# wq2012/SpectralCluster

Measured on AMD Instinct MI355X. Metric: predict() calls/sec, n=8192 d=256 ICASSP2018 (GraphCut, eigengap k in [2,20], cosine k-means), higher is better.
Workload: dtype f64; 1 GPU; icassp2018_graphcut_n8192_d256_k8_max20; n_samples=8192, n_features=256, parallelism=replicas x1, collectives=none

## Files before the change

### include/spectralcluster_amd.h

```cpp
#ifndef SPECTRALCLUSTER_AMD_H_
#define SPECTRALCLUSTER_AMD_H_

#include <stddef.h>
#include <stdint.h>

#ifdef __cplusplus
extern "C" {
#endif

#define SC_ABI_VERSION 11
#define SC_MAX_OPS 16
#define SC_MAX_BLUR_RADIUS 32
#define SC_MAX_EIG 128
#define SC_MAX_STAGES 16

typedef struct sc_handle_s* sc_handle;

typedef enum sc_status {
  SC_OK = 0,
  SC_ERR_INVALID = -1,
  SC_ERR_OOM = -2,
  SC_ERR_HIP = -3,
  SC_ERR_NOT_CONVERGED = -4,
  SC_ERR_UNSUPPORTED = -5,
// ... 134 lines not shown
enum { SC_MEM_HOST = 0, SC_MEM_DEVICE = 1 };
typedef struct sc_array {
  const void* data;
  int32_t dtype;
  int32_t location;
  int64_t rows, cols;
  int64_t row_stride;
  int64_t col_stride;
} sc_array;
int sc_array_layout(int* array_bytes, int* field_offsets);
int sc_device_count(void);
int sc_device_info(int device, char* name, int name_len, char* arch, int arch_len,
                   int* compute_units, int64_t* total_mem_bytes);

int sc_create(int device, sc_handle* out);
int sc_destroy(sc_handle h);
int sc_reserve(sc_handle h, int n_max, int d_max);
const char* sc_last_error(sc_handle h);
int sc_synchronize(sc_handle h);
void* sc_stream(sc_handle h);
int sc_set_profiling(sc_handle h, int level);
int sc_set_diffuse_mode(sc_handle h, int mode);
int sc_set_free_prune(sc_handle h, int on);

int sc_config_default(sc_config* cfg);
int sc_gaussian_weights(double sigma, int32_t* radius, double* weights);
int sc_set_blur_weights(sc_handle h, int radius, const double* weights);

int sc_predict(sc_handle h, const double* x, int n, int d, const sc_config* cfg,
               int64_t* labels, sc_diag* diag);

int sc_predict_array(sc_handle h, const sc_array* x, const sc_config* cfg, int64_t* labels,
                     sc_diag* diag);

int sc_set_embeddings(sc_handle h, const double* x, int n, int d);
int sc_set_embeddings_array(sc_handle h, const sc_array* x);
int sc_compute_affinity(sc_handle h);
int sc_set_affinity(sc_handle h, const double* affinity, int n);
int sc_set_affinity_array(sc_handle h, const sc_array* affinity);
int sc_predict_affinity_array(sc_handle h, const sc_array* affinity, const sc_config* cfg,
                              int64_t* labels, sc_diag* diag);
int sc_eig_ncluster(sc_handle h, const sc_config* cfg, sc_diag* diag);
int sc_num_eigenvalues(sc_handle h);
int sc_get_eigenvalues(sc_handle h, double* out, int count);
int sc_num_eigenvectors(sc_handle h);
int sc_get_eigenvectors(sc_handle h, double* out, int n, int ncols);
// ... 360 lines not shown
```

### spectralcluster_amd/_lib.py

```python

from __future__ import annotations

import ctypes
import os
import threading
import typing

import numpy as np

SC_MAX_OPS = 16
SC_MAX_BLUR_RADIUS = 32
SC_MAX_EIG = 128
SC_MAX_STAGES = 16

SC_OK = 0
SC_ERR_INVALID = -1
SC_ERR_OOM = -2
SC_ERR_HIP = -3
SC_ERR_NOT_CONVERGED = -4
SC_ERR_UNSUPPORTED = -5
SC_ERR_NON_FINITE = -6

STAGE_NAMES = ("affinity", "refine", "diffuse", "scaling", "eig", "kmeans",
               "total", "blur", "threshold_sym", "matvec", "affinity_gemm",
# ... 183 lines not shown

_c_int64_p = ctypes.POINTER(ctypes.c_int64)
_c_int_p = ctypes.POINTER(ctypes.c_int)
_handle_t = ctypes.c_void_p

PROTOTYPES = {
    "sc_abi_version": (ctypes.c_int, []),
    "sc_struct_sizes": (ctypes.c_int, [ctypes.POINTER(ctypes.c_int),
                                       ctypes.POINTER(ctypes.c_int)]),
    "sc_array_layout": (ctypes.c_int, [ctypes.POINTER(ctypes.c_int),
                                       ctypes.POINTER(ctypes.c_int)]),
    "sc_device_count": (ctypes.c_int, []),
    "sc_device_info": (ctypes.c_int, [ctypes.c_int, ctypes.c_char_p, ctypes.c_int,
                                      ctypes.c_char_p, ctypes.c_int, _c_int_p,
                                      _c_int64_p]),
    "sc_create": (ctypes.c_int, [ctypes.c_int, ctypes.POINTER(_handle_t)]),
    "sc_destroy": (ctypes.c_int, [_handle_t]),
    "sc_reserve": (ctypes.c_int, [_handle_t, ctypes.c_int, ctypes.c_int]),
    "sc_last_error": (ctypes.c_char_p, [_handle_t]),
    "sc_synchronize": (ctypes.c_int, [_handle_t]),
    "sc_set_profiling": (ctypes.c_int, [_handle_t, ctypes.c_int]),
    "sc_set_diffuse_mode": (ctypes.c_int, [_handle_t, ctypes.c_int]),
    "sc_set_free_prune": (ctypes.c_int, [_handle_t, ctypes.c_int]),
    "sc_stage_diffuse_rowstats": (ctypes.c_int, [_handle_t, _c_double_p, ctypes.c_int,
                                                 ctypes.c_int, _c_double_p, _c_double_p,
                                                 ctypes.POINTER(ctypes.c_int32)]),
    "sc_stage_block_operator": (ctypes.c_int, [_handle_t, ctypes.c_int,
                                               ctypes.POINTER(ctypes.c_int32),
                                               ctypes.POINTER(_c_double_p),
                                               ctypes.POINTER(_c_double_p),
                                               ctypes.POINTER(_c_double_p),
                                               ctypes.POINTER(_c_double_p),
                                               ctypes.POINTER(_c_double_p),
                                               ctypes.POINTER(_c_double_p), ctypes.c_int]),
    "sc_stage_krylov_state": (ctypes.c_int, [_handle_t, ctypes.POINTER(ctypes.c_int32),
                                             _c_double_p, _c_double_p, _c_double_p, _c_double_p,
                                             _c_double_p]),
    "sc_stage_front": (ctypes.c_int, [_handle_t, ctypes.c_int, ctypes.POINTER(ScConfig),
                                      ctypes.c_int, ctypes.POINTER(ctypes.c_int32), ctypes.c_int,
                                      ctypes.POINTER(_c_double_p), _c_double_p, _c_double_p,
                                      ctypes.POINTER(ScFrontOut)]),
    "sc_stage_tridiag": (ctypes.c_int, [_handle_t, _c_double_p, ctypes.c_int, _c_double_p,
                                        _c_double_p, _c_double_p, _c_double_p, _c_double_p,
                                        _c_double_p]),
    "sc_stage_tridiag_values": (ctypes.c_int, [_handle_t, _c_double_p, _c_double_p, ctypes.c_int,
                                               _c_double_p]),
# ... 561 lines not shown
```

### spectralcluster_amd/csrc/api.hip

```cpp
#include <algorithm>
#include <array>
#include <cmath>
#include <cstdio>
#include <cstdlib>
#include <cstring>
#include <vector>

#include <condition_variable>
#include <mutex>
#include <string>
#include <thread>

#include "handle.h"
#include "host_pool.h"

int ensure_matrices(sc_handle h, int n, int d, bool affinity_copy) {
  h->krylov_m = 0;
  h->arnoldi_m = 0;
  const size_t ldn = matrix_ld(n);
  const size_t nn = (size_t)n * ldn * sizeof(double);
  if (affinity_copy) SC_TRY(grow(h, h->A0, nn));
  SC_TRY(grow(h, h->B1, nn));
  SC_TRY(grow(h, h->B2, nn));
  if (d > 0) {
// ... 116 lines not shown
  hipDeviceProp_t prop;
  if (hipGetDeviceProperties(&prop, device) != hipSuccess) return SC_ERR_HIP;
  if (name && name_len > 0) snprintf(name, name_len, "%s", prop.name);
  if (arch && arch_len > 0) snprintf(arch, arch_len, "%s", prop.gcnArchName);
  if (compute_units) *compute_units = prop.multiProcessorCount;
  if (total_mem_bytes) *total_mem_bytes = (int64_t)prop.totalGlobalMem;
  return SC_OK;
}


extern "C" int sc_create(int device, sc_handle* out) {
  if (!out) return SC_ERR_INVALID;
  *out = nullptr;
  int count = 0;
  if (hipGetDeviceCount(&count) != hipSuccess || count <= 0) return SC_ERR_HIP;
  if (device < 0 || device >= count) return SC_ERR_INVALID;
  sc_handle h = new sc_handle_s();
  h->device = device;
  if (hipSetDevice(device) != hipSuccess ||
      hipStreamCreateWithFlags(&h->stream, hipStreamNonBlocking) != hipSuccess) {
    delete h;
    return SC_ERR_HIP;
  }
  const unsigned ev_flags = hipEventDisableSystemFence;
  for (int i = 0; i < 48; ++i) {
    if (hipEventCreateWithFlags(&h->ev[i], ev_flags) != hipSuccess) {
      delete h;
      return SC_ERR_HIP;
    }
  }
  if (hipHostMalloc(reinterpret_cast<void**>(&h->h_theta), 3 * kLdq * sizeof(double)) !=
          hipSuccess ||
      hipHostMalloc(reinterpret_cast<void**>(&h->h_flags), 16 * sizeof(int)) !=
          hipSuccess ||
      hipHostMalloc(reinterpret_cast<void**>(&h->h_rr),
                    (2 * kHostRRSingle * kHostRRSingle + 64) * sizeof(double)) != hipSuccess) {
    delete h;
    return SC_ERR_HIP;
  }
  *out = h;
  return SC_OK;
}

extern "C" int sc_destroy(sc_handle h) {
  if (!h) return SC_OK;
  for (sc_handle sub : h->pool) sc_destroy(sub);
  h->pool.clear();
  for (sc_handle sub : h->gslots) sc_destroy(sub);
  h->gslots.clear();
  for (sc_handle sub : h->gshort) sc_destroy(sub);
  h->gshort.clear();
  hipSetDevice(h->device);
  hipStreamSynchronize(h->stream);
  DevBuf* bufs[] = {&h->X,     &h->Xn,    &h->A0,     &h->B1,      &h->B2,    &h->rowmax,
                    &h->rowsum, &h->cvec,  &h->pvec,   &h->tvec,    &h->deg,   &h->blurw, &h->blur_tmp, &h->dvec, &h->cut, &h->rmpart, &h->splitk, &h->tilemap, &h->tilemap_table, &h->cropval, &h->statp, &h->crvec, &h->thetai, &h->Vre, &h->Vim, &h->gpart, &h->gsrc, &h->genL, &h->ahc_size, &h->ahc_chain, &h->ahc_Z, &h->ahc_lab, &h->ahc_cent, &h->fb_part, &h->fb_small, &h->sck_slots, &h->sck_part, &h->sck_rec, &h->sck_mats, &h->fb_x, &h->fb_cent, &h->fb_int, &h->Cq, &h->Cband, &h->Cpairs, &h->Cporig, &h->cp[0], &h->cp[1], &h->cp[2], &h->cp[3], &h->cp[4], &h->symflag,
                    &h->Q,     &h->Q2,    &h->Vs,     &h->W,       &h->partial, &h->T,
                    &h->Y,     &h->Yt,    &h->theta,  &h->resid,   &h->G,     &h->Rinv,
                    &h->Hbuf,  &h->hsq,   &h->colnorm, &h->flags,  &h->E,     &h->Ek,   &h->Eio,
                    &h->td_d,  &h->td_e,  &h->td_theta, &h->td_work, &h->td_tau, &h->td_panel, &h->mvsym,
                    &h->kXc,   &h->kxsq,  &h->kclosest, &h->kcand, &h->kenorm, &h->krnd,
                    &h->kcent, &h->klab32, &h->klab64, &h->kinfo, &h->kchain, &h->gkrnd, &h->gpack, &h->gypack, &h->ginfo, &h->glabels, &h->gjtab, &h->gsftab, &h->gswtab,
                    &h->kbig, &h->kbigw, &h->fq, &h->ft32, &h->fy1, &h->fR, &h->fscal, &h->fwords, &h->fcand, &h->fY, &h->fsplit, &h->fypart, &h->frpart, &h->fq2part, &h->fmx64, &h->ftau64, &h->fplan, &h->Xalt, &h->Xstage, &h->gneg};
  for (DevBuf* b : bufs)
    if (b->p) hipFree(b->p);
  for (DevBuf& b : h->kgen)
    if (b.p) hipFree(b.p);
  for (int i = 0; i < 48; ++i) hipEventDestroy(h->ev[i]);
  if (h->h_theta) hipHostFree(h->h_theta);
  if (h->h_flags) hipHostFree(h->h_flags);
  if (h->h_rr) hipHostFree(h->h_rr);
  if (h->h_free) hipHostFree(h->h_free);
  if (h->h_reduce) hipHostFree(h->h_reduce);
  if (h->h_sck) hipHostFree(h->h_sck);
  if (h->sync_ev) hipEventDestroy(h->sync_ev);
  for (int b = 0; b < kGroupBanks; ++b) {
    if (h->gbank_ev[b]) hipEventDestroy(h->gbank_ev[b]);
    if (h->gbank_stream[b]) hipStreamDestroy(h->gbank_stream[b]);
  }
  if (h->gchain_stream) hipStreamDestroy(h->gchain_stream);
  if (h->copy_stream) hipStreamDestroy(h->copy_stream);
  if (h->gcheck_ev) hipEventDestroy(h->gcheck_ev);
  for (sc_handle lane : h->glanes) sc_destroy(lane);
  h->glanes.clear();
  delete h->gpool;
  if (h->h_gpack) hipHostFree(h->h_gpack);
  if (h->h_gypack) hipHostFree(h->h_gypack);
  if (h->h_gjtab) hipHostFree(h->h_gjtab);
  if (h->h_gsftab) hipHostFree(h->h_gsftab);
  if (h->h_gswtab) hipHostFree(h->h_gswtab);
  if (h->gsftab_ev) hipEventDestroy(h->gsftab_ev);
  if (h->h_ginfo) hipHostFree(h->h_ginfo);
  if (h->h_glabels) hipHostFree(h->h_glabels);
  hipStreamDestroy(h->stream);
  delete h;
  return SC_OK;
}

extern "C" const char* sc_last_error(sc_handle h) { return h ? h->err.c_str() : ""; }

extern "C" int sc_synchronize(sc_handle h) {
  if (!h) return SC_ERR_INVALID;
  SC_HIP(h, hipStreamSynchronize(h->stream));
  return SC_OK;
}

extern "C" int sc_reserve(sc_handle h, int n_max, int d_max) {
  if (!h || n_max <= 0 || d_max < 0) return SC_ERR_INVALID;
  SC_HIP(h, hipSetDevice(h->device));
  SC_TRY(ensure_matrices(h, n_max, d_max));
  SC_TRY(ensure_eig(h, n_max));
  SC_TRY(ensure_kmeans(h, n_max));
  return SC_OK;
}

static double numpy_sum_short(const double* a, int n) {
// ... 334 lines not shown
  t.pending = false;
  if (!diag) return;
  float dms = 0.f;
  for (int i = 0; i < t.n_diffuse; ++i) dms += ev_ms(h, t.diffuse[i][0], t.diffuse[i][1]);
  diag->stage_ms[SC_STAGE_DIFFUSE] = dms;
  diag->stage_ms[SC_STAGE_REFINE] = ev_ms(h, t.begin, t.after_refine) - dms;
  diag->stage_ms[SC_STAGE_SCALING] = ev_ms(h, t.after_refine, t.after_scaling);
  diag->stage_ms[SC_STAGE_EIG] = ev_ms(h, t.after_scaling, t.after_eig);
  if (t.free_path) {
    diag->stage_ms[SC_STAGE_FREE_QUANTIZE] = ev_ms(h, h->free_ev[0], h->free_ev[1]);
    diag->stage_ms[SC_STAGE_FREE_PRODUCT] = ev_ms(h, h->free_ev[1], h->free_ev[2]);
    diag->stage_ms[SC_STAGE_FREE_SCAN] = ev_ms(h, h->free_ev[2], h->free_ev[3]);
    diag->stage_ms[SC_STAGE_FREE_STATS] = ev_ms(h, h->free_ev[3], h->free_ev[4]);
  }
  if (t.fine) {
    diag->stage_ms[SC_STAGE_BLUR] = ev_ms(h, t.blur[0], t.blur[1]);
    diag->stage_ms[SC_STAGE_THRESHOLD_SYM] = ev_ms(h, t.thr[0], t.thr[1]);
    float mv = 0.f;
    for (int i = 0; i < h->n_mv_ev; ++i) mv += ev_ms(h, h->mv_ev[i][0], h->mv_ev[i][1]);
    diag->stage_ms[SC_STAGE_MATVEC] = mv;
  }
}

int eig_ncluster_impl(sc_handle h, const sc_config* cfg, sc_diag* diag, FrontResult* front_only,
                      const FrontResult* resume, bool defer_timing,
                      FrontResult* stop_before_solver) {
  const int n = h->n, ld = h->ldn;
  hipStream_t s = h->stream;
  const double* cur = ptr<double>(h->A0);
  double* bufs[2] = {ptr<double>(h->B1), ptr<double>(h->B2)};
  int which = 0;
  bool symmetric = h->affinity_symmetric;
  const bool constrain_after = constraint_active(h, cfg, false);
  bool folded_rownorm = false;
  int e_begin, e_after_refine;
  const bool fine = h->profile_level >= 2;
  int eb0 = -1, eb1 = -1, et0 = -1, et1 = -1;
  h->n_mv_ev = 0;
  bool free_path = false;
  const double* amax_of = nullptr;
  const double* digits_of = nullptr;
  float diffuse_ms_events[SC_MAX_OPS][2];
  int n_diffuse = 0;
  ev_rec(h, &e_begin);
  const bool blur_fast = (cfg->blur_radius == 4 || cfg->blur_radius == 8) && n >= 128;
  const double* pending_diag = nullptr;
  bool have_partials = false;
  bool have_row_stats = false;
  int crop_source = 0, cut_kernel = 0;
  h->last_blur = BlurLaunch();
  if (resume) {
    cur = resume->matrix;
    symmetric = resume->symmetric;
    folded_rownorm = resume->folded_rownorm;
    which = resume->scratch == bufs[0] ? 0 : 1;
    if (resume->free_op) h->free_checked = false;
  }
  for (int i = 0; i < (resume ? 0 : cfg->n_ops); ++i) {
    const int op = cfg->ops[i];
    const int next = i + 1 < cfg->n_ops ? cfg->ops[i + 1] : 0;
    const int next2 = i + 2 < cfg->n_ops ? cfg->ops[i + 2] : 0;
    const bool thr_sym_fusable = true;
    const bool partials_usable = cfg->threshold_type == SC_THRESHOLD_ROW_MAX &&
                                 !cfg->preserve_diagonal;
    if (op == SC_OP_ROW_WISE_NORMALIZE && symmetric && i == cfg->n_ops - 1 &&
        !constrain_after) {
      folded_rownorm = true;
// ... 135 lines not shown
    double* out = bufs[which];
    which ^= 1;
    SC_TRY(adjust_affinity(h, cfg, cur, symmetric, out, n, ld));
    cur = out;
    symmetric = symmetric && h->constraint_symmetric;
    have_row_stats = false;
  }
  ev_rec(h, &e_after_refine);
  bool flags_by_kernel = false;
  if (resume) {
    SC_TRY(ensure_eig(h, n));
  } else if (!symmetric) {
    SC_TRY(ensure_gen(h, n));
    launch_row_stats(s, cur, n, ld, ptr<double>(h->rowmax), ptr<double>(h->deg));
    launch_scaling_general(s, ptr<double>(h->deg), n, cfg->laplacian_type,
                           ptr<double>(h->cvec), ptr<double>(h->crvec), ptr<double>(h->pvec));
  } else {
    if (!have_row_stats)
      launch_row_stats(s, cur, n, ld, ptr<double>(h->rowmax), ptr<double>(h->rowsum));
    SC_TRY(ensure_eig(h, n));
    launch_scaling_vectors(s, ptr<double>(h->rowmax), ptr<double>(h->rowsum), n,
                           cfg->laplacian_type, folded_rownorm ? 1 : 0, ptr<double>(h->cvec),
                           ptr<double>(h->pvec), ptr<double>(h->tvec), ptr<int>(h->flags),
                           h->affinity_from_embeddings ? ptr<int>(h->symflag) : nullptr);
    flags_by_kernel = true;
  }
  SC_TRY(ensure_eig(h, n));
  if (flags_by_kernel) {
  } else if (h->affinity_from_embeddings)
    SC_HIP(h, hipMemcpyAsync(ptr<int>(h->flags) + 12, ptr<int>(h->symflag) + 1, sizeof(int),
                             hipMemcpyDeviceToDevice, s));
  else
    SC_HIP(h, hipMemsetAsync(ptr<int>(h->flags) + 12, 0, sizeof(int), s));
  launch_check_finite(s, ptr<double>(h->cvec), ptr<double>(h->pvec), n, ptr<int>(h->flags) + 12);
  if (front_only && !flags_by_kernel)
    SC_HIP(h, hipMemsetAsync(ptr<int>(h->flags) + 13, 0, 3 * sizeof(int), s));
  SC_TRY(check_last(h, "scaling launch"));
  if (sw::eig_trace() > 2 && symmetric) {
    std::vector<double> rm(n), rs(n);
    hipMemcpyAsync(rm.data(), h->rowmax.p, n * sizeof(double), hipMemcpyDeviceToHost, s);
    hipMemcpyAsync(rs.data(), h->rowsum.p, n * sizeof(double), hipMemcpyDeviceToHost, s);
    hipStreamSynchronize(s);
    int imin = 0, imax = 0;
    for (int i = 0; i < n; ++i) {
      if (rm[i] < rm[imin]) imin = i;
      if (rm[i] > rm[imax]) imax = i;
    }
    fprintf(stderr, "[sc] scaling: fused stats %d; rowmax min %.6g at %d, max %.6g at %d; "
            "rowsum[%d] %.6g\n", (int)have_row_stats, rm[imin], imin, rm[imax], imax, imin,
            rs[imin]);
  }
  int e_after_scaling;
  ev_rec(h, &e_after_scaling);
  FrontResult op;
  op.matrix = cur;
  op.scratch = bufs[which];
  op.ld = ld;
  op.symmetric = symmetric;
  op.folded_rownorm = folded_rownorm;
  op.free_op = free_path || (resume && resume->free_op);
  op.laplacian_type = cfg->laplacian_type;
  op.chain_flags_cleared = flags_by_kernel;
  op.skip_fused = resume && resume->skip_fused;
  op.digits_fused = free_path && digits_of == cur;
  op.diffuse_explicit = !free_path && n_diffuse > 0;
  op.crop_source = crop_source;
  op.cut_kernel = cut_kernel;
  if (stop_before_solver) {
    *stop_before_solver = op;
    return SC_OK;
  }
  if (front_only) {
    *front_only = op;
    return SC_OK;
  }
  EigRequest rq = make_eig_request(cfg);
  EigDecision dc;
  std::vector<double> w;
  if (symmetric) {
    SC_TRY(sym_topk(h, op, n, rq, diag, &dc, &w));
  } else {
    rq.decision_aware = 1;
    SC_TRY(gen_topk(h, cur, ld, n, cfg->laplacian_type, rq, diag, &dc, &w, bufs[which]));
  }
  int e_after_eig;
  ev_rec(h, &e_after_eig);
  h->last_w = w;
  if (diag) {
    diag->n = n;
    diag->n_clusters_raw = dc.n_clusters_raw;
    diag->max_delta = dc.max_delta;
    diag->eig_descending = rq.descend;
    diag->n_eigenvalues = std::min((int)w.size(), SC_MAX_EIG);
    for (int i = 0; i < diag->n_eigenvalues; ++i) diag->eigenvalues[i] = w[i];
    diag->symmetry_state = !symmetric ? 3 : (folded_rownorm ? 2 : 1);
    if (!free_path && n_diffuse > 0) diag->diffuse_path = SC_DIFFUSE_PATH_EXPLICIT;
  }
  StageEvents& t = h->stage_events;
// ... 69 lines not shown
  sc_diag* dg = diag ? diag : &local;
  memset(dg, 0, sizeof(*dg));
  h->nev = 0;
  int e0, e1, e2;
  ev_rec(h, &e0);
  if (from_embeddings) SC_TRY(sc_compute_affinity(h));
  if (constraint_active(h, cfg, true)) SC_TRY(sc_apply_constraint(h, cfg));
  ev_rec(h, &e1);
  SC_TRY(eig_ncluster_impl(h, cfg, dg, nullptr, nullptr, true));
  int k = dg->n_clusters_raw;
  if (cfg->min_clusters > 0 && k < cfg->min_clusters) k = cfg->min_clusters;
  const int rc_cluster = sc_cluster(h, cfg, k, labels, dg);
  if (rc_cluster != SC_OK) {
    h->stage_events.pending = false;
    return rc_cluster;
  }
  ev_rec(h, &e2);
  SC_HIP(h, hipStreamSynchronize(h->stream));
  resolve_stage_times(h, dg);
  dg->stage_ms[SC_STAGE_AFFINITY] = ev_ms(h, e0, e1);
  dg->stage_ms[SC_STAGE_TOTAL] = ev_ms(h, e0, e2);
  if (h->profile_level >= 1 && from_embeddings)
    dg->stage_ms[SC_STAGE_AFFINITY_GEMM] = ev_ms(h, h->aff_ev[0], h->aff_ev[1]);
  return SC_OK;
}

extern "C" int sc_set_profiling(sc_handle h, int level) {
  if (!h || level < 0 || level > 2) return SC_ERR_INVALID;
  h->profile_level = level;
  return SC_OK;
}

std::vector<sc_array> host_f64_arrays(const double* const* xs, const int* ns, int d, int count) {
  std::vector<sc_array> arrays(std::max(count, 0));
  for (int i = 0; i < count; ++i) arrays[i] = host_f64_array(xs[i], ns[i], d);
  return arrays;
}

int predict_sequence(sc_handle h, const int* idx, int count, const sc_array* xs,
                     const int* ns, int d, const sc_config* cfg, int64_t* const* labels,
                     sc_diag* diags) {
  auto at = [&](int k) { return idx ? idx[k] : k; };
  auto one_call = [&](int i) -> int {
    SC_TRY(validate_config(h, cfg));
    SC_HIP(h, hipSetDevice(h->device));
    h->sweep_slot.clear();
// ... 374 lines not shown
```

### spectralcluster_amd/csrc/eig_driver.hip

```cpp
#include <ctime>

#include "handle.h"
#include "host_eig.h"
#include "host_pool.h"


static double value_error_bound(const double* theta, const double* resid, int m, int i,
                                bool symmetric) {
  const double r = resid[i];
  if (!symmetric || !(r > 0.0) || !std::isfinite(r)) return r;
  double delta = __builtin_huge_val();
  if (i > 0) delta = std::min(delta, theta[i - 1] - resid[i - 1] - theta[i]);
  if (i + 1 < m) delta = std::min(delta, theta[i] - theta[i + 1] - resid[i + 1]);
  else return r;
  delta -= r;
  if (!(delta > 0.0) || !std::isfinite(delta)) return r;
  return std::min(r, 2.0 * r * r / delta);
}

extern "C" int sc_host_value_error_bound(const double* theta, const double* resid, int m, int i,
                                         double* bound) {
  if (!theta || !resid || !bound || m < 1 || i < 0 || i >= m) return SC_ERR_INVALID;
  *bound = value_error_bound(theta, resid, m, i, true);
  return SC_OK;
// ... 332 lines not shown
  if (rq.fixed_count > 0 || rq.descend) return false;
  return rq.max_clusters == 0 || rq.eigengap_type == SC_EIGENGAP_NORMALIZED_DIFF;
}

static EigWorkspace eig_workspace(sc_handle h) {
  EigWorkspace ws;
  ws.Q = ptr<double>(h->Q);
  ws.Q2 = ptr<double>(h->Q2);
  ws.Vs = ptr<double>(h->Vs);
  ws.W = ptr<double>(h->W);
  ws.partial = ptr<double>(h->partial);
  ws.T = ptr<double>(h->T);
  ws.Y = ptr<double>(h->Y);
  ws.theta = ptr<double>(h->theta);
  ws.resid = ptr<double>(h->resid);
  ws.G = ptr<double>(h->G);
  ws.Rinv = ptr<double>(h->Rinv);
  ws.Hbuf = ptr<double>(h->Hbuf);
  ws.hsq = ptr<double>(h->hsq);
  ws.Yt = ptr<double>(h->Yt);
  ws.colnorm = ptr<double>(h->colnorm);
  ws.flags = ptr<int>(h->flags);
  return ws;
}

int sym_topk(sc_handle h, const FrontResult& op_in, int n, const EigRequest& rq_in,
             sc_diag* diag, EigDecision* out_dc, std::vector<double>* out_w) {
  hipStream_t s = h->stream;
  h->krylov_m = 0;
  h->arnoldi_m = 0;
  SC_TRY(ensure_eig(h, n));
  FrontResult op = op_in;
  const int ld = op.ld;
  auto free_materialize = [&](bool with_stats) -> int {
    if (!op.free_op) return SC_OK;
    if (op.scratch == nullptr || op.scratch == op.matrix)
      return fail(h, SC_ERR_UNSUPPORTED, "no scratch matrix to form the Diffuse product in");
    SC_TRY(ensure_tilemap(h, n));
    GemmRowStats rs{1, ptr<double>(h->statp), ptr<double>(h->statp) + (size_t)n * gemm_tile_dim(n),
                    ptr<double>(h->rowmax), ptr<double>(h->rowsum)};
    launch_gemm_nt(s, op.matrix, ld, op.matrix, ld, op.scratch, ld, n, n, n, kEpiNone, true,
                   ptr<double>(h->splitk), h->tilemap_cur, with_stats ? &rs : nullptr);
    SC_TRY(check_last(h, "diffuse launch"));
    double* a_buffer = const_cast<double*>(op.matrix);
    op.matrix = op.scratch;
    op.scratch = a_buffer;
// ... 78 lines not shown
                             hipMemcpyDeviceToHost, s));
    if (sw::eig_trace())
      SC_HIP(h, hipMemcpyAsync(h->h_flags + 1, ptr<int>(h->flags) + 1, 7 * sizeof(int),
                               hipMemcpyDeviceToHost, s));
    SC_HIP(h, hipStreamSynchronize(s));
    if (h->h_flags[12] != 0) return fail(h, SC_ERR_NON_FINITE, kNonFiniteMessage);
    trace_jacobi(h);
    for (int i = 0; i < n; ++i) h->h_theta[kLdq + i] = 0.0;
    dc = analyze(rq, h->h_theta, h->h_theta + kLdq, n, n, true);
    if (!dc.enough) return fail(h, SC_ERR_UNSUPPORTED, "eigen request cannot be satisfied");
    m = n;
    const int cols = n;
    launch_rowmajor_to_colmajor(s, ptr<double>(h->Y), kLdq, n, cols, ptr<double>(h->E),
                                round_up(n, 16));
    back_transform_cols(h, n, cols);
    h->n_vec = cols;
    if (diag) diag->eig_path = SC_EIG_PATH_DENSE_JACOBI;
    dc.kw = n;
  } else {
  restart_lanczos:
    m = 0;
    cycles = 0;
    bool done = false;
    uint64_t seed = 0x5eed5eedull;
    LzChain chain;
    if (dense && many_vectors) {
      SC_TRY(dense_fallback(5));
      done = true;
    }
    if (done) {
    } else if (fused) {
      if (!op.chain_flags_cleared)
        SC_HIP(h, hipMemsetAsync(ptr<int>(h->flags) + 13, 0, 3 * sizeof(int), s));
      op.chain_flags_cleared = false;
      const EigWorkspace ws = eig_workspace(h);
      chain = LzChain();
      chain.three_pass = three_pass;
      launch_lz_link(s, ws, &chain, n, 0, 0, 4, -1, cvec, 0, true, seed, false);
      launch_lz_link(s, ws, &chain, n, 0, 4, 3, -1, cvec, 0, false, 0, true);
      launch_lz_link(s, ws, &chain, n, 0, 3, 0, 0, cvec, 0, false, 0, false);
      SC_TRY(check_last(h, "start block launch"));
    } else {
      launch_random_block(s, ptr<double>(h->W), n, seed);
      SC_TRY(orthonormalize(h, n, 0, false, 0, 0, false, cvec));
      const int rc0 = finish_block(h, n, 0, 0, cvec, &seed);
      if (rc0 == SC_ERR_NOT_CONVERGED) {
        SC_TRY(dense_fallback(3));
        done = true;
      } else {
        SC_TRY(rc0);
      }
      SC_HIP(h, hipMemsetAsync(h->T.p, 0, (size_t)kLdq * kLdq * sizeof(double), s));
    }
    if (!done && sw::eig_force_dense()) {
      SC_TRY(dense_fallback(4));
      done = true;
    }
    const int cap = std::min(kEigBasisCap, ((n - kEigBlock) / kEigBlock) * kEigBlock);
    const int first_check = std::min(3 * kEigBlock, cap);
    auto check_due = [&](int mm) {
      return cycles == 0 ? (mm >= first_check && (mm <= 4 * kEigBlock ||
                                                  mm % (2 * kEigBlock) == 0 || mm + kEigBlock > cap))
// ... 1124 lines not shown
```

### spectralcluster_amd/csrc/handle.h

```cpp
#ifndef SPECTRALCLUSTER_AMD_HANDLE_H_
#define SPECTRALCLUSTER_AMD_HANDLE_H_

#include <algorithm>
#include <array>
#include <cmath>
#include <cstdio>
#include <cstdlib>
#include <cstring>
#include <string>
#include <vector>

#include "sc_internal.h"

using namespace sc;

struct DevBuf {
  void* p = nullptr;
  size_t bytes = 0;
};

constexpr int kKgenBufs = 12;
constexpr int kGroupBanks = 2;
constexpr int kGroupLanes = 3;

struct StageEvents {
  bool pending = false, fine = false, free_path = false;
  int begin = -1, after_refine = -1, after_scaling = -1, after_eig = -1;
  int diffuse[SC_MAX_OPS][2];
  int n_diffuse = 0;
  int blur[2] = {-1, -1}, thr[2] = {-1, -1};
};

struct sc_handle_s {
  int device = 0;
  hipStream_t stream = nullptr;
  std::string err;
  int n = 0, d = 0, ldn = 0, ldx = 0;
  bool have_x = false, have_affinity = false;
  bool have_cropval = false;
  int n_vec = 0;
  DevBuf X, Xn, A0, B1, B2;
  DevBuf Xalt;
  hipStream_t copy_stream = nullptr;
  DevBuf Xstage;
  DevBuf rowmax, rowsum, cvec, pvec, tvec, deg, dvec, cut, rmpart, splitk, tilemap;
  DevBuf cropval, statp;
  DevBuf Cq, cp[5], symflag;
  DevBuf Cband;
  bool have_constraint = false, constraint_symmetric = false, constraint_applied = false;
  bool constraint_banded = false;
  DevBuf Cpairs, Cporig;
  bool constraint_pairs = false;
  int pairs_count = 0;
  bool affinity_symmetric = true;
  bool affinity_from_embeddings = false;
  int qn = 0;
  int tilemap_nt = 0;
  DevBuf tilemap_table;
// ... 103 lines not shown
constexpr int kMaxCols = 128;
inline int matrix_ld(int n) {
  int ld = round_up(n, 16);
  if (ld % 512 == 0) ld += 16;
  return ld;
}


#define SC_HIP(h, call)                                                         \
  do {                                                                          \
    hipError_t e_ = (call);                                                     \
    if (e_ != hipSuccess) {                                                     \
      (h)->err = std::string(#call) + ": " + hipGetErrorString(e_);             \
      return e_ == hipErrorOutOfMemory ? SC_ERR_OOM : SC_ERR_HIP;               \
    }                                                                           \
  } while (0)

#define SC_TRY(expr)                \
  do {                              \
    int rc_ = (expr);               \
    if (rc_ != SC_OK) return rc_;   \
  } while (0)

inline int fail(sc_handle h, int code, const std::string& msg) {
  if (h) h->err = msg;
  return code;
}

inline int grow(sc_handle h, DevBuf& b, size_t bytes) {
  if (b.bytes >= bytes) return SC_OK;
  if (b.p) {
    SC_HIP(h, hipStreamSynchronize(h->stream));
    SC_HIP(h, hipFree(b.p));
    b.p = nullptr;
    b.bytes = 0;
  }
  SC_HIP(h, hipMalloc(&b.p, bytes));
  b.bytes = bytes;
  return SC_OK;
}
template <typename T>
inline T* ptr(const DevBuf& b) {
  return reinterpret_cast<T*>(b.p);
}

int ensure_matrices(sc_handle h, int n, int d, bool affinity_copy = true);
// ... 80 lines not shown
};

struct EigDecision {
  bool enough = false;
  bool converged = false;
  int kw = 0;
  int kvec = 0;
  int n_clusters_raw = 0;
  double max_delta = 0.0;
  double max_resid = 0.0;
  bool unsupported = false;
  int fail_kind = 0;
  int fail_index = -1;
};

struct FrontResult {
  const double* matrix = nullptr;
  double* scratch = nullptr;
  int ld = 0;
  bool symmetric = false, folded_rownorm = false;
  bool free_op = false;
  int laplacian_type = 0;
  bool chain_flags_cleared = false;
  bool skip_fused = false;
  bool digits_fused = false, diffuse_explicit = false;
  int crop_source = 0, cut_kernel = 0;
};
EigRequest make_eig_request(const sc_config* cfg);
int upload_blur_weights(sc_handle h, const sc_config* cfg);
int run_refine_op(sc_handle h, int op, const sc_config* cfg, const double* in, double* out, int n,
                  int ld);
int eig_ncluster_impl(sc_handle h, const sc_config* cfg, sc_diag* diag, FrontResult* front_only,
                      const FrontResult* resume = nullptr, bool defer_timing = false,
                      FrontResult* stop_before_solver = nullptr);
void kmeans_seed_constants(int k, double* u_first, int* trials, std::vector<double>* rnd);
KmeansWorkspace kmeans_workspace(sc_handle h);

struct GroupEigMember {
  sc_handle h = nullptr;
  const double* S = nullptr;
  int ld = 0, n = 0;
  EigRequest rq;
  int status = 0;
  EigDecision dc;
  std::vector<double> w;
  int basis = 0, passes = 0;
  bool skip_fused = false;
  bool free_op = false;
};
int sym_topk_group(sc_handle lead, GroupEigMember* mem, int count, bool want_vectors = true);
int dense_topk_group(sc_handle lead, GroupEigMember* mem, int count);
bool sym_group_eligible(int n, const EigRequest& rq, bool any_size = false);

int sym_topk(sc_handle h, const FrontResult& op, int n, const EigRequest& rq, sc_diag* diag,
             EigDecision* out_dc, std::vector<double>* out_w);
int gen_topk(sc_handle h, const double* M, int ld, int n, int laplacian_type,
             const EigRequest& rq, sc_diag* diag, EigDecision* out_dc,
             std::vector<double>* out_w, double* scratch);
int hessenberg_reduce_scaled(sc_handle h, double* B, int ld, int n, double* absmax, double* tau,
                             double* vwork, double* eig_scale);
void gen_residuals(hipStream_t s, const double* Q, const double* OpQ, int m, int n,
                   const double* Yre, const double* Yim, const double* theta_re,
                   const double* theta_im, int count, double* partial, double* resid);

bool free_diffuse_wanted(sc_handle h, const sc_config* cfg, int n, const EigRequest& rq,
                         bool in_group = false);
int free_group_prepare(sc_handle* hs, const double* const* A, const double* const* cuts,
                       const double* ps, int count, const int* lds, const int* ns, hipStream_t s,
                       double floor_value, struct FreeItem* items, struct TsDigits* digits);
int free_group_digits(sc_handle* hs, const struct FreeItem* items, int count, hipStream_t s);
int free_group_end(sc_handle* hs, const struct FreeItem* items, int count, hipStream_t s);
int free_fused_prepare(sc_handle h, hipStream_t s, int n, const double* cut, double p,
                       double floor_value);
void free_front_info(sc_handle h, int* candidates, int* overflow_rows, int* forms_s);
int free_diffuse_stats(sc_handle h, const double* A, int ld, int n, bool have_amax = false,
                       bool digits_ready = false);
// ... 60 lines not shown
```

### spectralcluster_amd/csrc/ingest.hip

```cpp
#include <climits>
#include <cstddef>

#include "handle.h"

namespace {

struct F16Bits { unsigned short v; };
struct BF16Bits { unsigned short v; };

__device__ __forceinline__ double widen(double v) { return v; }
__device__ __forceinline__ double widen(float v) { return (double)v; }
__device__ __forceinline__ double widen(BF16Bits b) {
  return (double)__uint_as_float((unsigned)b.v << 16);
}
__device__ __forceinline__ double widen(F16Bits b) {
  const unsigned h = b.v;
  const unsigned long long sign = (unsigned long long)(h >> 15) << 63;
  const unsigned e = (h >> 10) & 31u, m = h & 1023u;
  unsigned long long bits;
  if (e == 31u) {
    bits = sign | (0x7ffull << 52) | ((unsigned long long)m << 42);
  } else if (e != 0u) {
    bits = sign | ((unsigned long long)(e + 1008u) << 52) | ((unsigned long long)m << 42);
  } else {
// ... 594 lines not shown
  h->sweep_slot.clear();
  return ingest_embeddings(h, *x, true);
}

extern "C" int sc_set_embeddings(sc_handle h, const double* x, int n, int d) {
  if (!h) return SC_ERR_INVALID;
  if (!x || n <= 0 || d <= 0) return fail(h, SC_ERR_INVALID, "embeddings must be (n, d)");
  const sc_array a = host_f64_array(x, n, d);
  return sc_set_embeddings_array(h, &a);
}

extern "C" int sc_predict_array(sc_handle h, const sc_array* x, const sc_config* cfg,
                                int64_t* labels, sc_diag* diag) {
  if (!h) return SC_ERR_INVALID;
  SC_TRY(validate_config(h, cfg));
  SC_TRY(sc_set_embeddings_array(h, x));
  return sc_run_resident(h, cfg, labels, diag);
}

extern "C" int sc_predict(sc_handle h, const double* x, int n, int d, const sc_config* cfg,
                          int64_t* labels, sc_diag* diag) {
  if (!h) return SC_ERR_INVALID;
  SC_TRY(validate_config(h, cfg));
  SC_TRY(sc_set_embeddings(h, x, n, d));
  return sc_run_resident(h, cfg, labels, diag);
}

extern "C" int sc_stage_ingest(sc_handle h, const sc_array* x, double* out) {
  if (!h) return SC_ERR_INVALID;
  if (!out) return fail(h, SC_ERR_INVALID, "out is NULL");
  SC_TRY(sc_set_embeddings_array(h, x));
  return d2h_matrix(h, ptr<double>(h->X), h->ldx, h->n, h->d, out);
}

extern "C" int sc_predict_batch_arrays(sc_handle h, const sc_array* xs, int count,
                                       const sc_config* cfg, int64_t* const* labels,
                                       sc_diag* diags, int group, int streams) {
  if (!h) return SC_ERR_INVALID;
  if (!xs || !labels || count < 0) return fail(h, SC_ERR_INVALID, "NULL argument");
  SC_TRY(validate_config(h, cfg));
  SC_HIP(h, hipSetDevice(h->device));
  bool device_source = false;
  std::vector<int> ns;
  int d = 0;
  SC_TRY(validate_batch_arrays(h, xs, count, &ns, &d, &device_source));
  if (count == 0) {
    h->last_routes.clear();
    return SC_OK;
// ... 7 lines not shown
```

### spectralcluster_amd/csrc/rowops.hip

```cpp
#include <algorithm>
#include <cstring>

#include "dpp.h"
#include "sc_internal.h"

namespace sc {

constexpr int kRowThreads = 256;

__device__ __forceinline__ double wave_max(double v) {
#pragma unroll
  for (int o = 32; o > 0; o >>= 1) v = fmax(v, __shfl_xor(v, o));
  return v;
}
__device__ __forceinline__ double wave_sum(double v) {
#pragma unroll
  for (int o = 32; o > 0; o >>= 1) v += __shfl_xor(v, o);
  return v;
}
__device__ __forceinline__ double block_max(double v, double* sm) {
  v = wave_max(v);
  __syncthreads();
  if ((threadIdx.x & 63) == 0) sm[threadIdx.x >> 6] = v;
  __syncthreads();
// ... 660 lines not shown
  } else if (lap == SC_LAPLACIAN_GRAPH_CUT) {
    const double h = 1.0 / (sqrt(deg) + eps);
    cv = h * sa;
    pv = -((h * deg) * h);
  }
  *c = cv;
  *p = pv;
  *t = tv;
}
__device__ __forceinline__ void scaling_vectors_body(const double* __restrict__ rowmax,
                                                     const double* __restrict__ rowsum, int n,
                                                     int lap, int rownorm,
                                                     double* __restrict__ c,
                                                     double* __restrict__ p,
                                                     double* __restrict__ t) {
  const int i = blockIdx.x * blockDim.x + threadIdx.x;
  if (i >= n) return;
  scaling_vectors_row(rownorm ? rowmax[i] : 1.0, rowsum[i], lap, rownorm, c + i, p + i, t + i);
}
__global__ void k_scaling_vectors(const double* __restrict__ rowmax,
                                  const double* __restrict__ rowsum, int n,
                                  int lap, int rownorm, double* __restrict__ c,
                                  double* __restrict__ p, double* __restrict__ t,
                                  int* __restrict__ flags, int* __restrict__ symflag) {
  scaling_vectors_body(rowmax, rowsum, n, lap, rownorm, c, p, t);
  if (flags != nullptr && blockIdx.x == 0 && threadIdx.x == 0) {
    flags[12] = symflag != nullptr ? symflag[1] : 0;
    flags[13] = 0;
    flags[14] = 0;
    flags[15] = 0;
  }
}
__global__ void k_scaling_vectors_g(const GroupOf<FrontItem> g, int lap, int rownorm) {
  const FrontItem& a = g.s[blockIdx.y];
  const int i = blockIdx.x * blockDim.x + threadIdx.x;
  if (i >= a.n) return;
  scaling_vectors_body(a.rowmax, a.rowsum, a.n, lap, rownorm, a.cvec, a.pvec, a.tvec);
  if (!isfinite(a.cvec[i]) || !isfinite(a.pvec[i]) ||
      (i == 0 && a.symflag != nullptr && a.symflag[1] != 0))
    a.flags[12] = 1;
}

__global__ void k_check_finite(const double* __restrict__ a, const double* __restrict__ b,
                               int n, int* __restrict__ flag) {
  const int i = blockIdx.x * blockDim.x + threadIdx.x;
  if (i >= n) return;
  if (!isfinite(a[i]) || !isfinite(b[i])) *flag = 1;
}

constexpr int kShortFrontMatrix = kDenseMax * (kDenseMax + 1);
constexpr int kShortFrontLdsBytes = (kShortFrontMatrix + 3 * kDenseMax) * (int)sizeof(double);
__device__ __forceinline__ void short_front_tail(const ShortFrontItem& it, double* sf_lds,
                                                 int threshold_type, double mult, int binarize,
// ... 352 lines not shown
  const TsDigits dg{Q, pitch, t, scal, ypart, rpart, q2part, mx64};
  hipLaunchKernelGGL(k_threshold_symmetrize_digits, dim3(t * (t + 1) / 2), dim3(256), 0, s, in,
                     out, n, ld, cut, mult, binarize, symtype, t, preserve_diag, dg);
}
void launch_free_partials_reduce(hipStream_t s, const double* ypart, const int* rpart, int n,
                                 double* y1, double* R, double* scal, const FreeSegs& segs) {
  const int nblk = (n + kTsTile - 1) / kTsTile;
  hipLaunchKernelGGL(k_free_partials_reduce, dim3(nblk), dim3(256), 0, s, ypart, rpart, n,
                     nblk, y1, R, reinterpret_cast<unsigned long long*>(scal) + 2, segs);
}
void launch_row_normalize(hipStream_t s, const double* in, double* out, int n,
                          int ld) {
  hipLaunchKernelGGL(k_row_normalize, dim3(n), dim3(kRowThreads), 0, s, in, out, n,
                     ld);
}
void launch_row_stats(hipStream_t s, const double* in, int n, int ld,
                      double* rowmax, double* rowsum) {
  hipLaunchKernelGGL(k_row_stats, dim3(n), dim3(kRowThreads), 0, s, in, n, ld,
                     rowmax, rowsum);
}
void launch_scaling_vectors(hipStream_t s, const double* rowmax,
                            const double* rowsum, int n, int laplacian_type,
                            int row_normalized, double* c, double* p, double* t, int* flags,
                            int* symflag) {
  hipLaunchKernelGGL(k_scaling_vectors, dim3((n + 255) / 256), dim3(256), 0, s,
                     rowmax, rowsum, n, laplacian_type, row_normalized, c, p, t, flags, symflag);
}
static GroupOf<FrontItem> front_pack(const FrontItem* items, int count, int* nmax) {
  GroupOf<FrontItem> g;
  memset(&g, 0, sizeof(g));
  *nmax = 0;
  for (int z = 0; z < count; ++z) {
    g.s[z] = items[z];
    *nmax = std::max(*nmax, items[z].n);
  }
  return g;
}
void launch_front_begin_group(hipStream_t s, const FrontItem* items, int count,
                              bool normalize_rows, bool init_words) {
  int nmax;
  const GroupOf<FrontItem> g = front_pack(items, count, &nmax);
  if (nmax == 0) return;
  if (init_words) hipLaunchKernelGGL(k_front_words_init_g, dim3(count), dim3(64), 0, s, g);
  if (normalize_rows)
    hipLaunchKernelGGL(k_normalize_rows_g, dim3((nmax + 3) / 4, count), dim3(kRowThreads), 0, s,
                       g);
}
void launch_cut_percentile_group(hipStream_t s, const FrontItem* items, int count, int zero_diag) {
  int nmax;
// ... 103 lines not shown
```

### spectralcluster_amd/csrc/sc_internal.h

```cpp
#pragma once

#include <hip/hip_runtime.h>

#include "switches.h"
#include <stdint.h>

#include <mutex>
#include <string>
#include <vector>

#include "../../include/spectralcluster_amd.h"

namespace sc {

constexpr int kWave = 64;
constexpr int kEigBlock = 8;
constexpr int kEigBasisCap = 128;
constexpr int kLdq = kEigBasisCap + kEigBlock;
constexpr int kDenseMax = 128;
constexpr int kHostRR = 64;
constexpr int kHostRRSingle = kEigBasisCap;
constexpr int kGenMax = 64;
constexpr int kMaxVectors = 64;
constexpr int kProjBlocks = 128;
// ... 124 lines not shown
                          int preserve_diag);
void launch_symmetrize(hipStream_t s, const double* in, double* out, int n, int ld,
                       int type);

void launch_affinity_integration(hipStream_t s, const double* a, const double* q, double* out,
                                 int n, int ld, int type);
void launch_affinity_integration_band(hipStream_t s, const double* a, const double* band,
                                      double* out, int n, int ld, int type);
void launch_cp_band_product(hipStream_t s, const double* tt, const double* band, double* x,
                            int n, int ld);
void launch_cp_prepare(hipStream_t s, const double* a, const double* deg, double alpha,
                       double* p, double* t0, int n, int ld);
void launch_cp_adjust(hipStream_t s, const double* tqt, const double* a, double scale,
                      double* out, int n, int ld);
void launch_transpose(hipStream_t s, const double* in, double* out, int n, int ld);
void launch_symmetry_flag(hipStream_t s, const double* in, int n, int ld, int* flag);
void launch_row_normalize(hipStream_t s, const double* in, double* out, int n,
                          int ld);
void launch_row_stats(hipStream_t s, const double* in, int n, int ld,
                      double* rowmax, double* rowsum);
void launch_scaling_vectors(hipStream_t s, const double* rowmax,
                            const double* rowsum, int n, int laplacian_type,
                            int row_normalized, double* c, double* p, double* t,
                            int* flags = nullptr, int* symflag = nullptr);
void launch_laplacian(hipStream_t s, const double* in, double* out, int n, int ld,
                      int laplacian_type, double* deg_ws);
void launch_check_finite(hipStream_t s, const double* a, const double* b, int n, int* flag);

struct EigWorkspace {
  double* Q = nullptr;
  double* Q2 = nullptr;
  double* Vs = nullptr;
  double* W = nullptr;
  double* partial = nullptr;
  double* T = nullptr;
  double* Y = nullptr;
  double* theta = nullptr;
  double* resid = nullptr;
  double* G = nullptr;
  double* Rinv = nullptr;
  double* Hbuf = nullptr;
  double* hsq = nullptr;
  double* Yt = nullptr;
  double* colnorm = nullptr;
  int* flags = nullptr;
};

// ... 556 lines not shown
```

### spectralcluster_amd/csrc/switches.h

```cpp
#ifndef SPECTRALCLUSTER_AMD_SWITCHES_H_
#define SPECTRALCLUSTER_AMD_SWITCHES_H_

#include <cstdlib>
#include <cstring>

namespace sc {
namespace sw {

inline int eig_trace() {
  static const int v = getenv("SC_EIG_TRACE") ? std::max(1, atoi(getenv("SC_EIG_TRACE"))) : 0;
  return v;
}
inline bool kmeans_trace() {
  static const bool v = getenv("SC_KMEANS_TRACE") != nullptr;
  return v;
}
inline bool group_trace() {
  static const bool v = getenv("SC_GROUP_TRACE") != nullptr;
  return v;
}
inline bool eig_host_chain() {
  static const bool v = getenv("SC_EIG_HOST_CHAIN") != nullptr;
  return v;
}
// ... 29 lines not shown
  return v;
}
inline int diffuse_free_min_n_group() {
  static const int v =
      getenv("SC_DIFFUSE_FREE_MIN_N") ? atoi(getenv("SC_DIFFUSE_FREE_MIN_N")) : 1536;
  return v;
}
inline int gen_dense_max_n() {
  static const int v = getenv("SC_GEN_DENSE_MAX_N") ? atoi(getenv("SC_GEN_DENSE_MAX_N")) : 512;
  return v;
}
inline bool free_no_prune() {
  static const bool v = getenv("SC_FREE_NO_PRUNE") != nullptr;
  return v;
}
inline bool sweep_one_by_one() {
  static const bool v = getenv("SC_SWEEP_ONE_BY_ONE") != nullptr;
  return v;
}
inline bool short_front_memberwise() {
  static const bool v = getenv("SC_SHORT_FRONT_MEMBERWISE") != nullptr;
  return v;
}

}
}

#endif
```

Baseline: 384.9 calls/s.

## Hoist Lanczos start-block links onto an auxiliary stream overlapping embedding ingest

Adds an auxiliary HIP stream with fork/join events. During predict, the first two Lanczos start-block link kernels are enqueued on that stream before the embeddings are uploaded, so they can run concurrently with ingest and the affinity front end. The saved chain state is then reused by the eigen solver instead of relaunching those links, and the scaling-vectors kernel no longer clears the chain flags in that case. The aim is to take the start-block setup off the critical path. The cost is extra event record/wait traffic and more complex state tracking, with a join before the solver and fallbacks for dense, resume or three-pass paths.

```diff
diff --git a/include/spectralcluster_amd.h b/include/spectralcluster_amd.h
--- a/include/spectralcluster_amd.h
+++ b/include/spectralcluster_amd.h
@@ -180,6 +180,7 @@
 int sc_set_profiling(sc_handle h, int level);
 int sc_set_diffuse_mode(sc_handle h, int mode);
 int sc_set_free_prune(sc_handle h, int on);
+int sc_set_branch_overlap(sc_handle h, int on);
 
 int sc_config_default(sc_config* cfg);
 int sc_gaussian_weights(double sigma, int32_t* radius, double* weights);
diff --git a/spectralcluster_amd/_lib.py b/spectralcluster_amd/_lib.py
--- a/spectralcluster_amd/_lib.py
+++ b/spectralcluster_amd/_lib.py
@@ -229,6 +229,7 @@
     "sc_set_profiling": (ctypes.c_int, [_handle_t, ctypes.c_int]),
     "sc_set_diffuse_mode": (ctypes.c_int, [_handle_t, ctypes.c_int]),
     "sc_set_free_prune": (ctypes.c_int, [_handle_t, ctypes.c_int]),
+    "sc_set_branch_overlap": (ctypes.c_int, [_handle_t, ctypes.c_int]),
     "sc_stage_diffuse_rowstats": (ctypes.c_int, [_handle_t, _c_double_p, ctypes.c_int,
                                                  ctypes.c_int, _c_double_p, _c_double_p,
                                                  ctypes.POINTER(ctypes.c_int32)]),
diff --git a/spectralcluster_amd/csrc/api.hip b/spectralcluster_amd/csrc/api.hip
--- a/spectralcluster_amd/csrc/api.hip
+++ b/spectralcluster_amd/csrc/api.hip
@@ -162,6 +162,12 @@
     delete h;
     return SC_ERR_HIP;
   }
+  if (hipStreamCreateWithFlags(&h->aux_stream, hipStreamNonBlocking) != hipSuccess ||
+      hipEventCreateWithFlags(&h->aux_ev[0], hipEventDisableTiming) != hipSuccess ||
+      hipEventCreateWithFlags(&h->aux_ev[1], hipEventDisableTiming) != hipSuccess) {
+    delete h;
+    return SC_ERR_HIP;
+  }
   const unsigned ev_flags = hipEventDisableSystemFence;
   for (int i = 0; i < 48; ++i) {
     if (hipEventCreateWithFlags(&h->ev[i], ev_flags) != hipSuccess) {
@@ -192,6 +198,7 @@
   h->gshort.clear();
   hipSetDevice(h->device);
   hipStreamSynchronize(h->stream);
+  if (h->aux_stream) hipStreamSynchronize(h->aux_stream);
   DevBuf* bufs[] = {&h->X,     &h->Xn,    &h->A0,     &h->B1,      &h->B2,    &h->rowmax,
                     &h->rowsum, &h->cvec,  &h->pvec,   &h->tvec,    &h->deg,   &h->blurw, &h->blur_tmp, &h->dvec, &h->cut, &h->rmpart, &h->splitk, &h->tilemap, &h->tilemap_table, &h->cropval, &h->statp, &h->crvec, &h->thetai, &h->Vre, &h->Vim, &h->gpart, &h->gsrc, &h->genL, &h->ahc_size, &h->ahc_chain, &h->ahc_Z, &h->ahc_lab, &h->ahc_cent, &h->fb_part, &h->fb_small, &h->sck_slots, &h->sck_part, &h->sck_rec, &h->sck_mats, &h->fb_x, &h->fb_cent, &h->fb_int, &h->Cq, &h->Cband, &h->Cpairs, &h->Cporig, &h->cp[0], &h->cp[1], &h->cp[2], &h->cp[3], &h->cp[4], &h->symflag,
                     &h->Q,     &h->Q2,    &h->Vs,     &h->W,       &h->partial, &h->T,
@@ -231,6 +238,9 @@
   if (h->gsftab_ev) hipEventDestroy(h->gsftab_ev);
   if (h->h_ginfo) hipHostFree(h->h_ginfo);
   if (h->h_glabels) hipHostFree(h->h_glabels);
+  for (hipEvent_t e : h->aux_ev)
+    if (e) hipEventDestroy(e);
+  if (h->aux_stream) hipStreamDestroy(h->aux_stream);
   hipStreamDestroy(h->stream);
   delete h;
   return SC_OK;
@@ -611,9 +621,42 @@
   }
 }
 
+static int eig_ncluster_body(sc_handle h, const sc_config* cfg, sc_diag* diag,
+                             FrontResult* front_only, const FrontResult* resume, bool defer_timing,
+                             FrontResult* stop_before_solver);
+
+int hoist_start_links(sc_handle h, int n) {
+  h->start_hoisted = false;
+  if (!branch_overlap_on(h) || n <= kDenseMax || sw::eig_host_chain()) return SC_OK;
+  SC_HIP(h, hipSetDevice(h->device));
+  SC_TRY(ensure_eig(h, n));
+  if (hipStreamQuery(h->stream) != hipSuccess) {
+    (void)hipGetLastError();
+    SC_TRY(aux_fork(h));
+  }
+  h->aux_pending = true;
+  SC_TRY(enqueue_start_links(h, h->aux_stream, n, &h->start_chain));
+  h->start_hoisted = true;
+  h->start_n = n;
+  return SC_OK;
+}
+int drop_start_links(sc_handle h) {
+  h->start_hoisted = false;
+  return aux_join(h);
+}
 int eig_ncluster_impl(sc_handle h, const sc_config* cfg, sc_diag* diag, FrontResult* front_only,
                       const FrontResult* resume, bool defer_timing,
                       FrontResult* stop_before_solver) {
+  const int rc =
+      eig_ncluster_body(h, cfg, diag, front_only, resume, defer_timing, stop_before_solver);
+  h->start_hoisted = false;
+  const int rcj = aux_join(h);
+  return rc != SC_OK ? rc : rcj;
+}
+
+static int eig_ncluster_body(sc_handle h, const sc_config* cfg, sc_diag* diag,
+                             FrontResult* front_only, const FrontResult* resume, bool defer_timing,
+                             FrontResult* stop_before_solver) {
   const int n = h->n, ld = h->ldn;
   hipStream_t s = h->stream;
   const double* cur = ptr<double>(h->A0);
@@ -632,6 +675,10 @@
   float diffuse_ms_events[SC_MAX_OPS][2];
   int n_diffuse = 0;
   ev_rec(h, &e_begin);
+  if (h->start_hoisted && (h->start_n != n || front_only || resume || n <= kDenseMax)) {
+    SC_TRY(aux_join(h));
+    h->start_hoisted = false;
+  }
   const bool blur_fast = (cfg->blur_radius == 4 || cfg->blur_radius == 8) && n >= 128;
   const double* pending_diag = nullptr;
   bool have_partials = false;
@@ -813,7 +860,8 @@
     launch_scaling_vectors(s, ptr<double>(h->rowmax), ptr<double>(h->rowsum), n,
                            cfg->laplacian_type, folded_rownorm ? 1 : 0, ptr<double>(h->cvec),
                            ptr<double>(h->pvec), ptr<double>(h->tvec), ptr<int>(h->flags),
-                           h->affinity_from_embeddings ? ptr<int>(h->symflag) : nullptr);
+                           h->affinity_from_embeddings ? ptr<int>(h->symflag) : nullptr,
+                           !h->start_hoisted);
     flags_by_kernel = true;
   }
   SC_TRY(ensure_eig(h, n));
@@ -851,7 +899,8 @@
   op.folded_rownorm = folded_rownorm;
   op.free_op = free_path || (resume && resume->free_op);
   op.laplacian_type = cfg->laplacian_type;
-  op.chain_flags_cleared = flags_by_kernel;
+  op.chain_flags_cleared = flags_by_kernel && !h->start_hoisted;
+  op.start_hoisted = h->start_hoisted;
   op.skip_fused = resume && resume->skip_fused;
   op.digits_fused = free_path && digits_of == cur;
   op.diffuse_explicit = !free_path && n_diffuse > 0;
@@ -865,6 +914,7 @@
     *front_only = op;
     return SC_OK;
   }
+  SC_TRY(aux_join(h));
   EigRequest rq = make_eig_request(cfg);
   EigDecision dc;
   std::vector<double> w;
@@ -980,6 +1030,12 @@
   dg->stage_ms[SC_STAGE_TOTAL] = ev_ms(h, e0, e2);
   if (h->profile_level >= 1 && from_embeddings)
     dg->stage_ms[SC_STAGE_AFFINITY_GEMM] = ev_ms(h, h->aff_ev[0], h->aff_ev[1]);
+  return SC_OK;
+}
+
+extern "C" int sc_set_branch_overlap(sc_handle h, int on) {
+  if (!h || on < -1 || on > 1) return SC_ERR_INVALID;
+  h->branch_overlap = on;
   return SC_OK;
 }
 
diff --git a/spectralcluster_amd/csrc/eig_driver.hip b/spectralcluster_amd/csrc/eig_driver.hip
--- a/spectralcluster_amd/csrc/eig_driver.hip
+++ b/spectralcluster_amd/csrc/eig_driver.hip
@@ -378,6 +378,19 @@
   ws.colnorm = ptr<double>(h->colnorm);
   ws.flags = ptr<int>(h->flags);
   return ws;
+}
+
+static void start_links(hipStream_t s, const EigWorkspace& ws, LzChain* chain, int n,
+                        uint64_t seed) {
+  launch_lz_link(s, ws, chain, n, 0, 0, 4, -1, nullptr, 0, true, seed, false);
+  launch_lz_link(s, ws, chain, n, 0, 4, 3, -1, nullptr, 0, false, 0, true);
+}
+constexpr uint64_t kLanczosSeed = 0x5eed5eedull;
+int enqueue_start_links(sc_handle h, hipStream_t s, int n, LzChain* chain) {
+  SC_HIP(h, hipMemsetAsync(ptr<int>(h->flags) + 13, 0, 3 * sizeof(int), s));
+  *chain = LzChain();
+  start_links(s, eig_workspace(h), chain, n, kLanczosSeed);
+  return check_last(h, "start block launch");
 }
 
 int sym_topk(sc_handle h, const FrontResult& op_in, int n, const EigRequest& rq_in,
@@ -502,7 +515,7 @@
     m = 0;
     cycles = 0;
     bool done = false;
-    uint64_t seed = 0x5eed5eedull;
+    uint64_t seed = kLanczosSeed;
     LzChain chain;
     if (dense && many_vectors) {
       SC_TRY(dense_fallback(5));
@@ -510,14 +523,18 @@
     }
     if (done) {
     } else if (fused) {
-      if (!op.chain_flags_cleared)
-        SC_HIP(h, hipMemsetAsync(ptr<int>(h->flags) + 13, 0, 3 * sizeof(int), s));
+      const EigWorkspace ws = eig_workspace(h);
+      if (op.start_hoisted && !three_pass) {
+        chain = h->start_chain;
+      } else {
+        if (!op.chain_flags_cleared)
+          SC_HIP(h, hipMemsetAsync(ptr<int>(h->flags) + 13, 0, 3 * sizeof(int), s));
+        chain = LzChain();
+        chain.three_pass = three_pass;
+        start_links(s, ws, &chain, n, seed);
+      }
+      op.start_hoisted = false;
       op.chain_flags_cleared = false;
-      const EigWorkspace ws = eig_workspace(h);
-      chain = LzChain();
-      chain.three_pass = three_pass;
-      launch_lz_link(s, ws, &chain, n, 0, 0, 4, -1, cvec, 0, true, seed, false);
-      launch_lz_link(s, ws, &chain, n, 0, 4, 3, -1, cvec, 0, false, 0, true);
       launch_lz_link(s, ws, &chain, n, 0, 3, 0, 0, cvec, 0, false, 0, false);
       SC_TRY(check_last(h, "start block launch"));
     } else {
diff --git a/spectralcluster_amd/csrc/handle.h b/spectralcluster_amd/csrc/handle.h
--- a/spectralcluster_amd/csrc/handle.h
+++ b/spectralcluster_amd/csrc/handle.h
@@ -34,6 +34,13 @@
 struct sc_handle_s {
   int device = 0;
   hipStream_t stream = nullptr;
+  hipStream_t aux_stream = nullptr;
+  hipEvent_t aux_ev[2] = {nullptr, nullptr};
+  bool aux_pending = false;
+  int branch_overlap = -1;
+  bool start_hoisted = false;
+  int start_n = 0;
+  LzChain start_chain;
   std::string err;
   int n = 0, d = 0, ldn = 0, ldx = 0;
   bool have_x = false, have_affinity = false;
@@ -183,6 +190,24 @@
     if (rc_ != SC_OK) return rc_;   \
   } while (0)
 
+inline bool branch_overlap_on(sc_handle h) {
+  if (h->profile_level >= 2) return false;
+  return h->branch_overlap >= 0 ? h->branch_overlap != 0 : !sw::serial_branches();
+}
+inline int aux_fork(sc_handle h) {
+  SC_HIP(h, hipEventRecord(h->aux_ev[0], h->stream));
+  h->aux_pending = true;
+  SC_HIP(h, hipStreamWaitEvent(h->aux_stream, h->aux_ev[0], 0));
+  return SC_OK;
+}
+inline int aux_join(sc_handle h) {
+  if (!h->aux_pending) return SC_OK;
+  h->aux_pending = false;
+  SC_HIP(h, hipEventRecord(h->aux_ev[1], h->aux_stream));
+  SC_HIP(h, hipStreamWaitEvent(h->stream, h->aux_ev[1], 0));
+  return SC_OK;
+}
+
 inline int fail(sc_handle h, int code, const std::string& msg) {
   if (h) h->err = msg;
   return code;
@@ -309,6 +334,7 @@
   bool free_op = false;
   int laplacian_type = 0;
   bool chain_flags_cleared = false;
+  bool start_hoisted = false;
   bool skip_fused = false;
   bool digits_fused = false, diffuse_explicit = false;
   int crop_source = 0, cut_kernel = 0;
@@ -339,6 +365,9 @@
 int dense_topk_group(sc_handle lead, GroupEigMember* mem, int count);
 bool sym_group_eligible(int n, const EigRequest& rq, bool any_size = false);
 
+int enqueue_start_links(sc_handle h, hipStream_t s, int n, LzChain* chain);
+int hoist_start_links(sc_handle h, int n);
+int drop_start_links(sc_handle h);
 int sym_topk(sc_handle h, const FrontResult& op, int n, const EigRequest& rq, sc_diag* diag,
              EigDecision* out_dc, std::vector<double>* out_w);
 int gen_topk(sc_handle h, const double* M, int ld, int n, int laplacian_type,
diff --git a/spectralcluster_amd/csrc/ingest.hip b/spectralcluster_amd/csrc/ingest.hip
--- a/spectralcluster_amd/csrc/ingest.hip
+++ b/spectralcluster_amd/csrc/ingest.hip
@@ -640,8 +640,20 @@
                           int64_t* labels, sc_diag* diag) {
   if (!h) return SC_ERR_INVALID;
   SC_TRY(validate_config(h, cfg));
-  SC_TRY(sc_set_embeddings(h, x, n, d));
-  return sc_run_resident(h, cfg, labels, diag);
+  if (!x || n <= 0 || d <= 0) return fail(h, SC_ERR_INVALID, "embeddings must be (n, d)");
+  const sc_array a = host_f64_array(x, n, d);
+  SC_TRY(validate_array(h, &a));
+  SC_HIP(h, hipSetDevice(h->device));
+  h->sweep_slot.clear();
+  int rc = hoist_start_links(h, n);
+  if (rc == SC_OK) rc = ingest_embeddings(h, a, false);
+  const int rcj = aux_join(h);
+  if (rc == SC_OK) rc = rcj;
+  if (rc == SC_OK && hipStreamSynchronize(h->stream) != hipSuccess)
+    rc = fail(h, SC_ERR_HIP, "hipStreamSynchronize: upload");
+  if (rc == SC_OK) rc = sc_run_resident(h, cfg, labels, diag);
+  const int rcd = drop_start_links(h);
+  return rc != SC_OK ? rc : rcd;
 }
 
 extern "C" int sc_stage_ingest(sc_handle h, const sc_array* x, double* out) {
diff --git a/spectralcluster_amd/csrc/rowops.hip b/spectralcluster_amd/csrc/rowops.hip
--- a/spectralcluster_amd/csrc/rowops.hip
+++ b/spectralcluster_amd/csrc/rowops.hip
@@ -706,13 +706,16 @@
                                   const double* __restrict__ rowsum, int n,
                                   int lap, int rownorm, double* __restrict__ c,
                                   double* __restrict__ p, double* __restrict__ t,
-                                  int* __restrict__ flags, int* __restrict__ symflag) {
+                                  int* __restrict__ flags, int* __restrict__ symflag,
+                                  int clear_chain) {
   scaling_vectors_body(rowmax, rowsum, n, lap, rownorm, c, p, t);
   if (flags != nullptr && blockIdx.x == 0 && threadIdx.x == 0) {
     flags[12] = symflag != nullptr ? symflag[1] : 0;
-    flags[13] = 0;
-    flags[14] = 0;
-    flags[15] = 0;
+    if (clear_chain) {
+      flags[13] = 0;
+      flags[14] = 0;
+      flags[15] = 0;
+    }
   }
 }
 __global__ void k_scaling_vectors_g(const GroupOf<FrontItem> g, int lap, int rownorm) {
@@ -1111,9 +1114,10 @@
 void launch_scaling_vectors(hipStream_t s, const double* rowmax,
                             const double* rowsum, int n, int laplacian_type,
                             int row_normalized, double* c, double* p, double* t, int* flags,
-                            int* symflag) {
+                            int* symflag, bool clear_chain) {
   hipLaunchKernelGGL(k_scaling_vectors, dim3((n + 255) / 256), dim3(256), 0, s,
-                     rowmax, rowsum, n, laplacian_type, row_normalized, c, p, t, flags, symflag);
+                     rowmax, rowsum, n, laplacian_type, row_normalized, c, p, t, flags, symflag,
+                     clear_chain ? 1 : 0);
 }
 static GroupOf<FrontItem> front_pack(const FrontItem* items, int count, int* nmax) {
   GroupOf<FrontItem> g;
diff --git a/spectralcluster_amd/csrc/sc_internal.h b/spectralcluster_amd/csrc/sc_internal.h
--- a/spectralcluster_amd/csrc/sc_internal.h
+++ b/spectralcluster_amd/csrc/sc_internal.h
@@ -170,7 +170,8 @@
 void launch_scaling_vectors(hipStream_t s, const double* rowmax,
                             const double* rowsum, int n, int laplacian_type,
                             int row_normalized, double* c, double* p, double* t,
-                            int* flags = nullptr, int* symflag = nullptr);
+                            int* flags = nullptr, int* symflag = nullptr,
+                            bool clear_chain = true);
 void launch_laplacian(hipStream_t s, const double* in, double* out, int n, int ld,
                       int laplacian_type, double* deg_ws);
 void launch_check_finite(hipStream_t s, const double* a, const double* b, int n, int* flag);
diff --git a/spectralcluster_amd/csrc/switches.h b/spectralcluster_amd/csrc/switches.h
--- a/spectralcluster_amd/csrc/switches.h
+++ b/spectralcluster_amd/csrc/switches.h
@@ -75,6 +75,10 @@
   static const bool v = getenv("SC_SHORT_FRONT_MEMBERWISE") != nullptr;
   return v;
 }
+inline bool serial_branches() {
+  static const bool v = getenv("SC_SERIAL_BRANCHES") != nullptr;
+  return v;
+}
 
 }
 }
```

After: 389.4 calls/s (median of 5 runs). +1.2%, better.
